# leo-stan/torch-points3d

Measured on AMD Instinct MI355X. Metric: point-clouds/sec fwd+bwd PointNet++SSG B=32 N=16384, higher is better.
Workload: dtype f32; 1 GPU; PointNet++ SSG (unet_3_ss) train step fwd+bwd+Adam, B=32 per GPU, N=16384, FEAT=3, 10 classes, pos~U[-1,1]^3 (BASELINE configs[1]); launch=hip-graph replay; geometry of step i+1 on a 2nd stream during step i, global_batch=32, points=16384, parallelism=dp1, whole clouds per rank, one flat gradient all-reduce (RCCL) per step

## Files before the change

### include/tp3d_hip.h

```cpp
#ifndef TP3D_HIP_H
#define TP3D_HIP_H

#include <stddef.h>
#include <stdint.h>

#ifdef __cplusplus
extern "C" {
#endif

#define TP3D_OK 0
#define TP3D_E_BADARG (-1)
#define TP3D_E_LAUNCH (-2)
#define TP3D_E_UNSORTED (-3)
#define TP3D_E_TOOBIG (-4)

#define TP3D_ABI_VERSION 39

int tp3d_abi_version(void);
const char *tp3d_strerror(int code);
int tp3d_last_hip_error(void);

#define TP3D_FPS_MAX_REG_POINTS 32768
int tp3d_fps_f32(const float *xyz, int B, int N, int npoint, float *scratch, int64_t *out_idx, void *stream);

// ... 272 lines not shown
                        float min_dist, float *dist2, int64_t *idx, void *workspace, size_t workspace_bytes, void *stream);
size_t tp3d_fgr_workspace_bytes(int64_t N);
int tp3d_fgr_accumulate_f32(const float *xyz, const float *xyz_target, int64_t N, int iter, void *workspace,
                            size_t workspace_bytes, void *stream);
int tp3d_fgr_solve(int64_t N, int iter, double mu_init, float *T, void *workspace, size_t workspace_bytes, void *stream);

int tp3d_segment_tile_rows(void);
int tp3d_segment_sum_chunk(void);
int tp3d_segment_transform_f32(const float *x, const float *T, const int64_t *seg, int64_t N, int64_t B, int k, int C, int ldx,
                               int ldo, int transpose, float *out, void *stream);
size_t tp3d_segment_transform_wgrad_workspace_bytes(int64_t N, int64_t B, int k);
int tp3d_segment_transform_wgrad_f32(const float *x, const float *dy, const int64_t *seg, int64_t N, int64_t B, int k, int ldx,
                                     int lddy, float *dT, void *workspace, size_t workspace_bytes, void *stream);
int tp3d_segment_bcast_cat_f32(const float *x, const float *g, const int64_t *seg, int64_t N, int64_t B, int C1, int C2, int ldx,
                               int ldg, int ldo, float *out, void *stream);
size_t tp3d_segment_sum_workspace_bytes(int64_t N, int64_t B, int C);
int tp3d_segment_sum_f32(const float *rows, const int64_t *seg, const float *scale, int64_t N, int64_t B, int col0, int C, int ld,
                         float *out, void *workspace, size_t workspace_bytes, void *stream);

#define TP3D_BOX_NMS_MAX_BOXES 4096
int tp3d_box_nms_max_boxes(void);
int tp3d_box_nms_f32(const float *boxes, const int64_t *classes, const int64_t *order, int B, int P, float overlap_threshold,
                     uint8_t *keep, void *stream);
int tp3d_box3d_iou_f64(const float *corners1, const float *corners2, int64_t n, int64_t m, double *iou, void *stream);
int tp3d_box_best_gt_f64(const float *det_corners, const int64_t *det_class, const int64_t *det_scene, int64_t D,
                         const float *gt_corners, const int64_t *gt_class, const int64_t *gt_scene_start, int64_t G, int64_t S,
                         double *ovmax, int64_t *jmax, void *stream);
int tp3d_ap_match(const int64_t *order, const int64_t *det_class, const int64_t *det_scene, int64_t D, const double *ovmax,
                  const int64_t *jmax, int64_t G, const double *thresholds, int T, uint8_t *taken, uint8_t *tp, void *stream);

int tp3d_gemm_tn_plan(int64_t M, int N, int K, int64_t *plan);
int tp3d_gemm_tn_x3_plan(int64_t M, int N, int K, int64_t *plan);
int tp3d_gemm_rows_plan(int64_t M, int N, int K, int64_t *plan);
int tp3d_bn_plan(int64_t M, int C, int pooled_ns, int64_t *plan);
int tp3d_scatter_plan(int B, int L, int nbins, int with_weights, int64_t *plan);

#ifdef __cplusplus
}
#endif
#endif
```

### torch_points3d_amd/_lib.py

```python
import collections
import ctypes
import os

import torch

from . import build as _build

_p = ctypes.c_void_p
_i = ctypes.c_int
_l = ctypes.c_int64
_f = ctypes.c_float

SIGNATURES = {
    "tp3d_fps_f32": [_p, _i, _i, _i, _p, _p, _p],
    "tp3d_ball_query_dense_f32": [_p, _p, _i, _i, _i, _f, _i, _i, _p, _p, _p, ctypes.c_size_t, _p],
    "tp3d_ball_query_partial_dense_f32": [_p, _p, _p, _p, _l, _l, _f, _i, _i, _p, _p, _p, _i, _i, _p, ctypes.c_size_t,
                                          _i, _p],
    "tp3d_three_nn_f32": [_p, _p, _i, _i, _i, _p, _p, _p],
    "tp3d_three_interpolate_fwd_f32": [_p, _p, _p, _i, _i, _i, _i, _p, _p],
    "tp3d_three_interpolate_bwd_f32": [_p, _p, _p, _i, _i, _i, _i, _p, _p, ctypes.c_size_t, _p],
    "tp3d_group_fwd_f32": [_p, _p, _i, _i, _i, _i, _i, _p, _p],
    "tp3d_group_bwd_f32": [_p, _p, _i, _i, _i, _i, _i, _p, _p, ctypes.c_size_t, _p],
    "tp3d_group_concat_fwd_f32": [_p, _p, _p, _p, _i, _i, _i, _i, _i, _i, _f, _i, _p, _p],
    "tp3d_rows_scatter_bwd_f32": [_p, _p, _p, _i, _i, _i, _i, _i, _i, _i, _p, _p, ctypes.c_size_t, _p],
# ... 54 lines not shown
    "tp3d_rsconv_msgmax_bwd_f32": [_p, _p, _p, _i, _p, _i, _p, _p, _l, _l, _l, _i, _p, _p, _p],
    "tp3d_sparse_set_build_i32": [_p, _l, _i, _i, _p, _p, _p, _p, _p, ctypes.c_size_t, _p],
    "tp3d_sparse_set_build_clouds_i32": [_p, _l, _i, _i, _i, _p, _p, _p, _p, _p, ctypes.c_size_t, _p],
    "tp3d_sparse_kmap_i32": [_p, _l, _i, _i, _i, _p, _p, _p, _l, _p, _p],
    "tp3d_sparse_kmap_mirror_i32": [_p, _l, _i, _p, _p],
    "tp3d_sparse_conv_f32": [_p, _p, _p, _l, _l, _i, _i, _i, _i, _p, _p],
    "tp3d_sparse_wgrad_f32": [_p, _p, _p, _l, _l, _i, _i, _i, _p, _p, ctypes.c_size_t, _p],
    "tp3d_sparse_conv_wide_f32": [_p, _p, _p, _l, _l, _i, _i, _i, _p, _p],
    "tp3d_sparse_wgrad_wide_f32": [_p, _p, _p, _l, _l, _i, _i, _i, _p, _p, ctypes.c_size_t, _p],
    "tp3d_scale_fuse_fwd_f32": [_p, _i, _l, _i, _i, _f, _p, _p, _p, _p, _p],
    "tp3d_scale_fuse_bwd_f32": [_p, _i, _l, _i, _i, _f, _p, _p, _p, _p, _p, _p],
    "tp3d_pv_quantize_f32": [_p, _l, _i, _p, _p],
    "tp3d_pv_trilinear_f32": [_p, _p, _l, _l, _i, _i, _p, _p],
    "tp3d_pv_invert_i32": [_p, _l, _i, _l, _p, _p, _p, ctypes.c_size_t, _p],
    "tp3d_pv_gather_f32": [_p, _p, _p, _p, _l, _i, _l, _i, _p, _p],
    "tp3d_pv_runsum_f32": [_p, _p, _p, _p, _p, _l, _i, _l, _i, _p, _p],
    "tp3d_cluster_voxel_mean_fwd_f32": [_p, _i, _p, _p, _p, _l, _l, _l, _i, _p, _p],
    "tp3d_cluster_voxel_mean_bwd_f32": [_p, _p, _p, _p, _p, _l, _l, _l, _i, _p, _p],
    "tp3d_region_grow_f32": [_p, _p, _p, _l, _p, _i, _f, _l, _p, _p, _p, _p, _p, _p, _p, ctypes.c_size_t, _p],
    "tp3d_feature_nn_f32": [_p, _p, _p, _p, _l, _l, _i, _f, _p, _p, _p, ctypes.c_size_t, _p],
    "tp3d_fgr_accumulate_f32": [_p, _p, _l, _i, _p, ctypes.c_size_t, _p],
    "tp3d_fgr_solve": [_l, _i, ctypes.c_double, _p, _p, ctypes.c_size_t, _p],
    "tp3d_segment_transform_f32": [_p, _p, _p, _l, _l, _i, _i, _i, _i, _i, _p, _p],
    "tp3d_segment_transform_wgrad_f32": [_p, _p, _p, _l, _l, _i, _i, _i, _p, _p, ctypes.c_size_t, _p],
    "tp3d_segment_bcast_cat_f32": [_p, _p, _p, _l, _l, _i, _i, _i, _i, _i, _p, _p],
    "tp3d_segment_sum_f32": [_p, _p, _p, _l, _l, _i, _i, _i, _p, _p, ctypes.c_size_t, _p],
    "tp3d_box_nms_f32": [_p, _p, _p, _i, _i, _f, _p, _p],
    "tp3d_box3d_iou_f64": [_p, _p, _l, _l, _p, _p],
    "tp3d_box_best_gt_f64": [_p, _p, _p, _l, _p, _p, _p, _l, _l, _p, _p, _p],
    "tp3d_ap_match": [_p, _p, _p, _l, _p, _p, _l, _p, _i, _p, _p, _p],
    "tp3d_gemm_tn_plan": [_l, _i, _i, _p],
    "tp3d_gemm_tn_x3_plan": [_l, _i, _i, _p],
    "tp3d_gemm_rows_plan": [_l, _i, _i, _p],
    "tp3d_bn_plan": [_l, _i, _i, _p],
    "tp3d_scatter_plan": [_i, _i, _i, _i, _p],
}
_z = ctypes.c_size_t
MISC = {
    "tp3d_abi_version": (_i, []),
    "tp3d_strerror": (ctypes.c_char_p, [_i]),
    "tp3d_last_hip_error": (_i, []),
    "tp3d_scatter_workspace_bytes": (_z, [_i, _i, _i, _i]),
    "tp3d_bn_workspace_floats": (_z, [_l, _i]),
    "tp3d_gemm_tn_workspace_floats": (_z, [_l, _i, _i]),
    "tp3d_gemm_tn_x3_workspace_floats": (_z, [_l, _i, _i]),
    "tp3d_gemm_tn_x3_serves": (_i, [_l, _i, _i]),
    "tp3d_gemm_tn_x3_red_chunks": (_i, [_l, _i, _i]),
    "tp3d_kpconv_bwd_workspace_bytes": (_z, [_l, _l]),
    "tp3d_gemm_rows_stat_floats": (_z, [_l, _i]),
    "tp3d_gemm_rows_stat_chunks": (_i, [_l, _i]),
    "tp3d_gemm_rows_narrow_chunks": (_i, [_l]),
    "tp3d_gemm_tn_bn_narrow_serves": (_i, [_l, _i, _i]),
    "tp3d_gemm_tn_bn_narrow_workspace_floats": (_z, [_l, _i, _i]),
    "tp3d_gemm_rows_bnbwd_sp_serves": (_i, [_l, _i, _i]),
    "tp3d_gemm_rows_x3_chunks": (_i, [_l, _i, _i, _i]),
    "tp3d_gemm_rows_sp_chunks": (_i, [_l, _i, _i, _i]),
    "tp3d_gemm_rows_workspace_floats": (_z, [_l, _i, _i]),
    "tp3d_kpconv_grad_workspace_bytes": (_z, [_l, _l, _i]),
    "tp3d_knn_workspace_bytes": (_z, [_i, _l, _i]),
    "tp3d_voxel_workspace_bytes": (_z, [_l]),
    "tp3d_ball_query_workspace_bytes": (_z, [_i, _l, _i]),
    "tp3d_sparse_workspace_bytes": (_z, [_l]),
    "tp3d_sparse_cloud_limit_max": (_i, []),
    "tp3d_sparse_wgrad_chunks": (_i, [_l, _i, _i, _i]),
    "tp3d_sparse_wgrad_workspace_floats": (_z, [_l, _i, _i, _i]),
    "tp3d_sparse_conv_wide_serves": (_i, [_i, _i, _i]),
# ... 225 lines not shown
```

### torch_points3d_amd/csrc/gemm_rows.hip

```cpp
#include <algorithm>

#include "tp3d_common.h"

namespace tp3d {

typedef float f32x16 __attribute__((ext_vector_type(16)));

constexpr int GR_BLOCK_T = 256;
constexpr int GR_BM = 128, GR_BK = 32;
constexpr int GR_LD = GR_BK + 4;

struct RowsEpilogue {
    const float *mean, *scale, *beta;
    float slope;
};

template <bool WIDE, int STATS>
__global__ __launch_bounds__(GR_BLOCK_T, 1) void gemm_rows_kernel(const float *__restrict__ A, const float *__restrict__ Bt,
                                                                int64_t M, int N, int K, int kchunk, int tiles_n,
                                                                int64_t items, float *__restrict__ C,
                                                                float *__restrict__ partial, RowsEpilogue epi)
{
    constexpr int BN = WIDE ? 128 : 64;
    constexpr int WR = WIDE ? 2 : 4;
    constexpr int WM = WIDE ? 2 : 1;
    constexpr int WN = 2;
    constexpr int PB = BN * (GR_BK / 4) / GR_BLOCK_T;
    __shared__ __attribute__((aligned(16))) float sA[GR_BM * GR_LD];
    __shared__ __attribute__((aligned(16))) float sB[BN * GR_LD];

    const int tid = threadIdx.x, lane = tid & 63, wave = tid >> 6;
    const int wr = WIDE ? wave >> 1 : wave, wc = WIDE ? wave & 1 : 0;
    const int l31 = lane & 31, lh = lane >> 5;
    const int kbeg = blockIdx.y * kchunk, kend = min(K, kbeg + kchunk);
    const int ksteps = (kend - kbeg + GR_BK - 1) / GR_BK;
    if (blockIdx.y > 0) C += (size_t)blockIdx.y * (size_t)M * N;

    auto decode = [&](int64_t item, int64_t &m0, int &n0, int64_t &rb) __attribute__((always_inline)) {
        const int64_t grp = item / (8 * tiles_n);
        const int rem = (int)(item % (8 * tiles_n));
        rb = grp * 8 + (rem & 7);
        m0 = rb * GR_BM;
// ... 314 lines not shown
                        pr[(size_t)N] = s2;
                        pr[(size_t)2 * N] = k;
                        pr[(size_t)3 * N] = (float)valid;
                    }
                }
            }
            if (STATS == 2) {
                if (valid > 0) have_shift = true;
                run_rows += valid;
            }
        }
        item = next_item;
        m0 = nm0;
        n0 = nn0;
        rb = nrb;
    }
    if (STATS == 2) {
        const int per = 8 * tiles_n;
        const int64_t slot = (int64_t)(blockIdx.x / per) * 8 + (blockIdx.x & 7);
#pragma unroll
        for (int j = 0; j < 2; ++j) {
            const int n = n0_first + (wc * 2 + j) * 32 + l31;
            if (lh == 0 && n < N) {
                float *pr = partial + ((size_t)(slot * 2 + wr) * 4) * N + n;
                pr[0] = run1[j];
                pr[(size_t)N] = run2[j];
                pr[(size_t)2 * N] = kshift[j];
                pr[(size_t)3 * N] = (float)run_rows;
            }
        }
    }
}


__global__ __launch_bounds__(256) void gemm_rows_sum_slabs_kernel(const float *__restrict__ slabs, int S, int64_t MN4,
                                                                   float *__restrict__ out, int N, RowsEpilogue epi)
{
    for (int64_t e = (int64_t)blockIdx.x * 256 + threadIdx.x; e < MN4; e += (int64_t)gridDim.x * 256) {
        float4 t = reinterpret_cast<const float4 *>(slabs)[e];
        for (int s = 1; s < S; ++s) {
            const float4 v = reinterpret_cast<const float4 *>(slabs + (size_t)s * MN4 * 4)[e];
            t.x += v.x;
            t.y += v.y;
            t.z += v.z;
            t.w += v.w;
        }
        if (epi.mean) {
            const int n = (int)((e * 4) % N);
            const float4 mu = *reinterpret_cast<const float4 *>(epi.mean + n), sc = *reinterpret_cast<const float4 *>(epi.scale + n);
            const float4 be = *reinterpret_cast<const float4 *>(epi.beta + n);
            t.x = (t.x - mu.x) * sc.x + be.x, t.y = (t.y - mu.y) * sc.y + be.y;
            t.z = (t.z - mu.z) * sc.z + be.z, t.w = (t.w - mu.w) * sc.w + be.w;
            t.x = t.x > 0.0f ? t.x : t.x * epi.slope, t.y = t.y > 0.0f ? t.y : t.y * epi.slope;
            t.z = t.z > 0.0f ? t.z : t.z * epi.slope, t.w = t.w > 0.0f ? t.w : t.w * epi.slope;
        }
        reinterpret_cast<float4 *>(out)[e] = t;
    }
}

}

using namespace tp3d;

namespace {
constexpr int GR_GRID = 1024;
struct RowsPlan {
    bool wide;
    int tiles_n, wave_rows;
    int64_t row_blocks, items, blocks;
    bool per_workgroup;
    int64_t chunks;
    int ksplit, kchunk;
};
RowsPlan rows_plan(int64_t M, int N, int K = 0, bool allow_split = false)
{
    RowsPlan p;
    const int rem = N % 128;
    p.wide = !(rem > 0 && rem <= 64);
    const int bn = p.wide ? 128 : 64;
    p.wave_rows = p.wide ? 2 : 4;
    p.tiles_n = (N + bn - 1) / bn;
    p.row_blocks = (M + GR_BM - 1) / GR_BM;
    const int64_t groups = (p.row_blocks + 7) / 8;
    p.items = groups * 8 * p.tiles_n;
    p.blocks = p.items < GR_GRID ? p.items : GR_GRID;
    p.per_workgroup = p.blocks == GR_GRID && GR_GRID % (8 * p.tiles_n) == 0;
    p.chunks = p.wave_rows * (p.per_workgroup ? GR_GRID / p.tiles_n : p.row_blocks);
    p.ksplit = 1;
    p.kchunk = K > 0 ? (K + GR_BK - 1) / GR_BK * GR_BK : 0;
    if (allow_split && K >= 1024 && p.items <= 128) {
        const int want = (int)((512 + p.items - 1) / p.items);
        const int by_k = K / 128;
        int s = want < by_k ? want : by_k;
        if (s > 16) s = 16;
        if (s > 1) {
            p.kchunk = ((K + s - 1) / s + GR_BK - 1) / GR_BK * GR_BK;
            p.ksplit = (K + p.kchunk - 1) / p.kchunk;
        }
    }
    return p;
}

template <bool WIDE>
int launch_rows(const RowsPlan &p, const float *A, const float *Bt, int64_t M, int N, int K, float *C, float *stat_partial,
                const RowsEpilogue &epi, hipStream_t s)
{
    const dim3 grid((unsigned)p.blocks, (unsigned)p.ksplit), block(GR_BLOCK_T);
    if (WIDE && p.ksplit == 1) {
        if (stat_partial && p.per_workgroup)
            hipLaunchKernelGGL(gemm_rows_wide_kernel<2>, grid, block, 0, s, A, Bt, M, N, K, p.tiles_n, p.items, C, stat_partial, epi);
        else if (stat_partial)
            hipLaunchKernelGGL(gemm_rows_wide_kernel<1>, grid, block, 0, s, A, Bt, M, N, K, p.tiles_n, p.items, C, stat_partial, epi);
        else
            hipLaunchKernelGGL(gemm_rows_wide_kernel<0>, grid, block, 0, s, A, Bt, M, N, K, p.tiles_n, p.items, C, stat_partial, epi);
        return check_launch();
    }
    if (stat_partial && p.per_workgroup)
        hipLaunchKernelGGL((gemm_rows_kernel<WIDE, 2>), grid, block, 0, s, A, Bt, M, N, K, p.kchunk, p.tiles_n, p.items,
                           C, stat_partial, epi);
    else if (stat_partial)
        hipLaunchKernelGGL((gemm_rows_kernel<WIDE, 1>), grid, block, 0, s, A, Bt, M, N, K, p.kchunk, p.tiles_n, p.items,
                           C, stat_partial, epi);
    else
        hipLaunchKernelGGL((gemm_rows_kernel<WIDE, 0>), grid, block, 0, s, A, Bt, M, N, K, p.kchunk, p.tiles_n, p.items,
                           C, stat_partial, epi);
    return check_launch();
}

int launch_rows_any(const RowsPlan &p, const float *A, const float *Bt, int64_t M, int N, int K, float *C,
                    float *stat_partial, const RowsEpilogue &epi, hipStream_t s)
{
    return p.wide ? launch_rows<true>(p, A, Bt, M, N, K, C, stat_partial, epi, s)
                  : launch_rows<false>(p, A, Bt, M, N, K, C, stat_partial, epi, s);
}

int rows_gemm(const float *A, const float *Bt, int64_t M, int N, int K, float *C, float *stat_partial, float *workspace,
              const RowsEpilogue &epi, hipStream_t s)
{
    const RowsEpilogue none = {nullptr, nullptr, nullptr, 1.0f};
    const RowsPlan p = rows_plan(M, N, K, !stat_partial && workspace && ((M * (int64_t)N) & 3) == 0 && (!epi.mean || (N & 3) == 0));
// ... 14 lines not shown
    const int64_t rows = p.chunks > by_block ? p.chunks : by_block;
    return (size_t)rows * 4 * (size_t)N;
}

TP3D_EXPORT int tp3d_gemm_rows_stat_chunks(int64_t M, int N)
{
    if (M <= 0 || N <= 0) return 0;
    return (int)rows_plan(M, N).chunks;
}

TP3D_EXPORT size_t tp3d_gemm_rows_workspace_floats(int64_t M, int N, int K)
{
    if (M <= 0 || N <= 0 || K <= 0) return 0;
    const RowsPlan p = rows_plan(M, N, K, true);
    return p.ksplit > 1 ? (size_t)p.ksplit * (size_t)M * (size_t)N : 0;
}

TP3D_EXPORT int tp3d_gemm_rows_plan(int64_t M, int N, int K, int64_t *plan)
{
    if (M <= 0 || N <= 0 || K < 0 || !plan) return TP3D_E_BADARG;
    const RowsPlan p = rows_plan(M, N, K, K > 0);
    plan[0] = p.tiles_n;
    plan[1] = p.row_blocks;
    plan[2] = p.items;
    plan[3] = p.blocks;
    plan[4] = p.chunks;
    plan[5] = p.per_workgroup ? 1 : 0;
    plan[6] = p.wave_rows;
    plan[7] = p.ksplit;
    plan[8] = p.wide ? 128 : 64;
    return TP3D_OK;
}

TP3D_EXPORT int tp3d_gemm_rows_f32(const float *A, const float *Bt, int64_t M, int N, int K, float *C, float *stat_partial,
                                   float *workspace, void *stream)
{
    if (M < 0 || N <= 0 || K <= 0 || (K & 3)) return TP3D_E_BADARG;
    if (M == 0) return TP3D_OK;
    if (!A || !Bt || !C) return TP3D_E_BADARG;
    const RowsEpilogue none = {nullptr, nullptr, nullptr, 1.0f};
    return rows_gemm(A, Bt, M, N, K, C, stat_partial, workspace, none, (hipStream_t)stream);
}

TP3D_EXPORT int tp3d_gemm_rows_epi_f32(const float *A, const float *Bt, int64_t M, int N, int K, const float *mean,
                                       const float *scale, const float *beta, float slope, float *C, float *workspace,
                                       void *stream)
{
    if (M < 0 || N <= 0 || K <= 0 || (K & 3)) return TP3D_E_BADARG;
    if (M == 0) return TP3D_OK;
    if (!A || !Bt || !C || !mean || !scale || !beta) return TP3D_E_BADARG;
    const RowsEpilogue epi = {mean, scale, beta, slope};
    return rows_gemm(A, Bt, M, N, K, C, nullptr, workspace, epi, (hipStream_t)stream);
}
```

### torch_points3d_amd/csrc/gemm_tn.hip

```cpp
#include <type_traits>

#include "tp3d_common.h"

namespace tp3d {

typedef float f32x16 __attribute__((ext_vector_type(16)));

constexpr int TN_BLOCK = 256;
constexpr int TN_BR_MAX = 64;

template <int WM, int WN, bool VECY, bool VECA, int GN = 2>
__global__ __launch_bounds__(TN_BLOCK) void gemm_tn_partial_kernel(const float *__restrict__ dY,
                                                                    const float *__restrict__ A, int64_t M, int N,
                                                                    int K, int64_t rows_per_split, int tiles_k,
                                                                    float *__restrict__ partial )
{
    constexpr int GK = 4 / GN;
    constexpr int TN = GN * WM * 32, TK = GK * WN * 32;
    constexpr int TN_BR = (WM * WN) % 3 == 0 ? 16 : 64 / (WM * WN);
    constexpr int LDN = TN + 4, LDK = TK + 4;
    __shared__ __attribute__((aligned(16))) float sY[TN_BR * LDN];
    __shared__ __attribute__((aligned(16))) float sA[TN_BR * LDK];

    const int tile = blockIdx.x;
    const int n0 = (tile / tiles_k) * TN, k0 = (tile % tiles_k) * TK;
    const int split = blockIdx.y;
    const int64_t r_begin = (int64_t)split * rows_per_split;
    const int64_t r_end = min(r_begin + rows_per_split, M);
    const int tid = threadIdx.x, lane = tid & 63, wave = tid >> 6;
    const int wr = wave / GK, wc = wave % GK;
    const int l31 = lane & 31, lh = lane >> 5;
    f32x16 acc[WM][WN];
#pragma unroll
    for (int i = 0; i < WM; ++i)
#pragma unroll
        for (int j = 0; j < WN; ++j)
#pragma unroll
            for (int e = 0; e < 16; ++e) acc[i][j][e] = 0.0f;


    auto load4 = [&](const float *base, int64_t r, int c, int ld, auto aligned_tag) __attribute__((always_inline)) -> float4 {
        constexpr bool aligned = decltype(aligned_tag)::value;
// ... 67 lines not shown
#pragma unroll
            for (int e = 0; e < 16; ++e) {
                const int n = n0 + (wr * WM + i) * 32 + (e & 3) + 8 * (e >> 2) + 4 * lh;
                const int k = k0 + (wc * WN + j) * 32 + l31;
                if (n < N && k < K) out[(size_t)n * K + k] = acc[i][j][e];
            }
}

constexpr int RD_E = 64, RD_S = 16;
__global__ __launch_bounds__(RD_E *RD_S) void gemm_tn_reduce_kernel(const float *__restrict__ partial, int S,
                                                                     int64_t NK, float *__restrict__ out)
{
    __shared__ float sm[RD_S][RD_E];
    const int tx = threadIdx.x % RD_E, ty = threadIdx.x / RD_E;
    const int64_t e = (int64_t)blockIdx.x * RD_E + tx;
    float acc = 0.0f;
    if (e < NK)
        for (int s = ty; s < S; s += RD_S) acc += partial[(size_t)s * NK + e];
    sm[ty][tx] = acc;
    __syncthreads();
    if (ty == 0 && e < NK) {
        float t = 0.0f;
#pragma unroll
        for (int k = 0; k < RD_S; ++k) t += sm[k][tx];
        out[e] = t;
    }
}

int tn_reduce_splits(const float *partial, int splits, int64_t NK, float *out, hipStream_t s)
{
    hipLaunchKernelGGL(gemm_tn_reduce_kernel, dim3((unsigned)((NK + RD_E - 1) / RD_E)), dim3(RD_E * RD_S), 0, s, partial, splits,
                       NK, out);
    return check_launch();
}

struct TnPlan {
    int wm, wn, gn, tn, tk, tiles_n, tiles_k, splits;
    int64_t rows_per_split;
};

static TnPlan plan_tn(int64_t M, int N, int K)
{
    TnPlan p;
    p.wm = N > 64 ? 2 : 1;
    if (K <= 64) p.wn = 1;
    else if (K <= 128) p.wn = 2;
    else if (K <= 192) p.wn = 3;
    else p.wn = ((K + 191) / 192) * 192 < ((K + 127) / 128) * 128 ? 3 : 2;
    p.gn = 2;
    if (N <= 32 && K >= 128) {
        p.gn = 1;
        p.wm = 1;
        p.wn = 1;
    }
    p.tn = 32 * p.gn * p.wm;
    p.tk = 32 * (4 / p.gn) * p.wn;
    p.tiles_n = (N + p.tn - 1) / p.tn;
    p.tiles_k = (K + p.tk - 1) / p.tk;
    const int tiles = p.tiles_n * p.tiles_k;
    int64_t want = (1024 + tiles - 1) / tiles;
    const int min_rows = 256;
    int64_t max_by_rows = (M + min_rows - 1) / min_rows;
    int64_t s = want < max_by_rows ? want : max_by_rows;
    if (s < 1) s = 1;
    if (s > 512) s = 512;
    p.rows_per_split = ((M + s - 1) / s + TN_BR_MAX - 1) / TN_BR_MAX * TN_BR_MAX;
    p.splits = (int)((M + p.rows_per_split - 1) / p.rows_per_split);
    return p;
}

static int launch_tn(const float *dY, const float *A, int64_t M, int N, int K, float *out, float *workspace, hipStream_t s)
{
    const TnPlan p = plan_tn(M, N, K);
    if (p.splits > 65535) return TP3D_E_TOOBIG;
    dim3 grid(p.tiles_n * p.tiles_k, p.splits);
    const bool vy = (N & 3) == 0, va = (K & 3) == 0;
#define TP3D_TN_LAUNCH(WM_, WN_, VY_, VA_)                                                                          \
    hipLaunchKernelGGL((gemm_tn_partial_kernel<WM_, WN_, VY_, VA_>), grid, dim3(TN_BLOCK), 0, s, dY, A, M, N, K,        \
                       p.rows_per_split, p.tiles_k, workspace)
#define TP3D_TN_ALIGN(WM_, WN_)                                                                                     \
    do {                                                                                                            \
        if (vy && va) TP3D_TN_LAUNCH(WM_, WN_, true, true);                                                         \
        else if (vy) TP3D_TN_LAUNCH(WM_, WN_, true, false);                                                         \
        else if (va) TP3D_TN_LAUNCH(WM_, WN_, false, true);                                                         \
        else TP3D_TN_LAUNCH(WM_, WN_, false, false);                                                                \
    } while (0)
    if (p.gn == 1) {
        if (vy && va) hipLaunchKernelGGL((gemm_tn_partial_kernel<1, 1, true, true, 1>), grid, dim3(TN_BLOCK), 0, s, dY, A, M, N, K,
                                         p.rows_per_split, p.tiles_k, workspace);
        else if (va) hipLaunchKernelGGL((gemm_tn_partial_kernel<1, 1, false, true, 1>), grid, dim3(TN_BLOCK), 0, s, dY, A, M, N, K,
                                        p.rows_per_split, p.tiles_k, workspace);
        else if (vy) hipLaunchKernelGGL((gemm_tn_partial_kernel<1, 1, true, false, 1>), grid, dim3(TN_BLOCK), 0, s, dY, A, M, N, K,
                                        p.rows_per_split, p.tiles_k, workspace);
        else hipLaunchKernelGGL((gemm_tn_partial_kernel<1, 1, false, false, 1>), grid, dim3(TN_BLOCK), 0, s, dY, A, M, N, K,
                                p.rows_per_split, p.tiles_k, workspace);
    } else if (p.wm == 2 && p.wn == 3) TP3D_TN_ALIGN(2, 3);
    else if (p.wn == 3) TP3D_TN_ALIGN(1, 3);
    else if (p.wm == 2 && p.wn == 2) TP3D_TN_ALIGN(2, 2);
    else if (p.wm == 2) TP3D_TN_ALIGN(2, 1);
    else if (p.wn == 2) TP3D_TN_ALIGN(1, 2);
    else TP3D_TN_ALIGN(1, 1);
// ... 42 lines not shown
```

### torch_points3d_amd/fused.py

```python
import collections

import torch
import torch.nn as nn

from . import _lib


USE_ROWS_GEMM = True


def _cl(x):
    return x.transpose(1, 2).contiguous()


def _pad4(c):
    return (c + 3) & ~3


def _slope_of(act):
    if act is None:
        return 1.0
    if isinstance(act, nn.LeakyReLU):
        return float(act.negative_slope)
    if isinstance(act, nn.ReLU):
# ... 74 lines not shown
    _lib.call("tp3d_gemm_tn_bn_narrow_f32", _lib.ptr(Y), _lib.ptr(dY_src), _lib.ptr(ls[0]), _lib.ptr(ls[2]),
              _lib.ptr(ls[3]), _lib.ptr(red[2]), _lib.ptr(red[3]), slope, _lib.ptr(A0), M, C, Kp, _lib.ptr(dW),
              _lib.ptr(nws), reverse, st)
    return dW


def gemm_tn(dY, A, x3=None, act=None, reverse=0):
    dY, A = dY.contiguous(), A.contiguous()
    M, N = dY.shape
    K = A.shape[1]
    terms = WGRAD_X3 if x3 is None else x3
    kernel = "x3" if terms and M > 0 and _lib.load().tp3d_gemm_tn_x3_serves(M, N, K) else "tn"
    if act is not None:
        if kernel != "x3":
            raise ValueError("gemm_tn(act=): only the bf16-pipe contraction forms its A operand (shape %s x %s x %s)" % (M, N, K))
        kernel = "x3_act"
    return _gemm_tn_launch(kernel, dY, A, terms, act, reverse)


def _gemm_tn_launch(kernel, dY, A, terms, act, reverse):
    dev = dY.device
    M, N = dY.shape
    K = A.shape[1]
    out = torch.empty((N, K), dtype=torch.float32, device=dev)
    ws = _lib.gemm_tn_workspace(M, N, K, dev, x3=kernel != "tn")
    with _lib.on_device(dev):
        if kernel == "x3_act":
            _lib.call("tp3d_gemm_tn_x3_act_f32", _lib.ptr(dY), _lib.ptr(A), _lib.ptr(act[0]), _lib.ptr(act[1]), _lib.ptr(act[2]),
                      float(act[3]), M, N, K, int(terms), _lib.ptr(out), _lib.ptr(ws), int(reverse), _lib.stream_ptr(dev))
        elif kernel == "x3":
            _lib.call("tp3d_gemm_tn_x3_f32", _lib.ptr(dY), _lib.ptr(A), M, N, K, int(terms), _lib.ptr(out), _lib.ptr(ws), int(reverse),
                      _lib.stream_ptr(dev))
        else:
            _lib.call("tp3d_gemm_tn_f32", _lib.ptr(dY), _lib.ptr(A), M, N, K, _lib.ptr(out), _lib.ptr(ws),
                      _lib.stream_ptr(dev))
    return out


SKINNY_MAX = 32
SKINNY_MIN_ROWS = 32768


def gemm_skinny(A, W):
    dev = A.device
    A, W = A.contiguous(), W.contiguous()
    M, K = A.shape
    N = W.shape[0]
    Y = torch.empty((M, N), dtype=torch.float32, device=dev)
    with _lib.on_device(dev):
        _lib.call("tp3d_gemm_skinny_f32", _lib.ptr(A), _lib.ptr(W), M, N, K, K, _lib.ptr(Y), _lib.stream_ptr(dev))
    return Y


def _is_skinny(M, a, b):
    return M >= SKINNY_MIN_ROWS and a <= SKINNY_MAX and b <= SKINNY_MAX


def gemm_rows(A, Bt, want_stats=False):
    dev = A.device
    M, K = A.shape
    N = Bt.shape[0]
    Bm = Bt.contiguous()
    C = torch.empty((M, N), dtype=torch.float32, device=dev)
    part, slabs = None, None
    h = _lib.load()
    if want_stats:
        part = _lib.workspace("gemm_rows_stats", 4 * h.tp3d_gemm_rows_stat_floats(M, N), dev)
    else:
        n = h.tp3d_gemm_rows_workspace_floats(M, N, K)
        if n:
            slabs = _lib.workspace("gemm_rows_slabs", 4 * n, dev)
    with _lib.on_device(dev):
        _lib.call("tp3d_gemm_rows_f32", _lib.ptr(A), _lib.ptr(Bm), M, N, K, _lib.ptr(C), _lib.ptr(part), _lib.ptr(slabs),
                  _lib.stream_ptr(dev))
    return C, part


def _finalize_stats(part, M, C, gamma, beta, bn, dev, st, chunks=None):
    stats = torch.empty((4, C), dtype=torch.float32, device=dev)
    if chunks is None:
        chunks = _lib.load().tp3d_gemm_rows_stat_chunks(M, C)
    _lib.call("tp3d_bn_finalize_f32", _lib.ptr(part), chunks, M, C, float(bn.eps),
              float(bn.momentum), _lib.ptr(gamma), _lib.ptr(beta), _lib.ptr(bn.running_mean), _lib.ptr(bn.running_var),
              _lib.ptr(bn.num_batches_tracked), _lib.ptr(stats[0]), _lib.ptr(stats[1]), _lib.ptr(stats[2]), _lib.ptr(stats[3]), st)
    _note_training_pass(bn)
    return stats


def _note_training_pass(bn):
    bn._tp3d_train_passes = getattr(bn, "_tp3d_train_passes", 0) + 1


_replay_epoch = 0


def note_graph_replay():
    global _replay_epoch
    _replay_epoch += 1


def eval_state_key(tensors, bns):
    return (tuple((t.data_ptr(), t._version) for t in tensors)
            + tuple(getattr(bn, "_tp3d_train_passes", 0) for bn in bns) + (_replay_epoch,))


ROWS_GEMM_MIN_COLS = 32
ROWS_GEMM_WITHOUT_STATS = True
ROWS_GEMM_EPILOGUE = True
ROWS_GEMM_NARROW = True
CHAIN_MIN_ROWS = 32768


def _rows_gemm_serves(cout):
    if not USE_ROWS_GEMM or cout < ROWS_GEMM_MIN_COLS:
        return False
    return ROWS_GEMM_NARROW or not (0 < cout % 128 <= 64)


def _bn_stats(Y, M, C, gamma, beta, bn, training, dev, st, bias=None):
    key = None
    if not training:
        key = eval_state_key((gamma, beta, bn.running_mean, bn.running_var) + ((bias,) if bias is not None else ()), (bn,))
        hit = getattr(bn, "_tp3d_eval_stats", None)
        if hit is not None and hit[0] == key:
            return hit[1]
    stats = torch.empty((4, C), dtype=torch.float32, device=dev)
    ws = _lib.bn_workspace(M, C, dev)
    _lib.call("tp3d_bn_stats_f32", _lib.ptr(Y), M, C, float(bn.eps), float(bn.momentum), _lib.ptr(gamma), _lib.ptr(beta),
              _lib.ptr(bn.running_mean), _lib.ptr(bn.running_var), _lib.ptr(bn.num_batches_tracked) if training else None,
              int(training), _lib.ptr(stats[0]), _lib.ptr(stats[1]), _lib.ptr(stats[2]), _lib.ptr(stats[3]), _lib.ptr(ws), st)
    if training:
        _note_training_pass(bn)
    if key is not None:
        if bias is not None:
            stats[0].sub_(bias.detach())
        bn._tp3d_eval_stats = (key, stats)
# ... 37 lines not shown
    want_stats = training and _lib.load().tp3d_gemm_rows_workspace_floats(M, Cout, Kp) == 0
    if rows and ROWS_GEMM_EPILOGUE and not training and not pool_ns and ROWS_GEMM_WITHOUT_STATS and not want_grad:
        return "rows_epi", False
    if rows and (want_stats or ROWS_GEMM_WITHOUT_STATS):
        return "rows", want_stats
    if skinny:
        return "skinny", False
    return "library", False


class _LinearBNAct(torch.autograd.Function):

    @staticmethod
    def forward(ctx, A, weight, gamma, beta, bn, slope, pool_ns, grad_enabled, bias=None):
        dev = A.device
        A = A.contiguous()
        M, Kp = A.shape
        Cout = weight.shape[0]
        W2 = weight.reshape(Cout, -1)
        Cin = W2.shape[1]
        if Kp != Cin:
            W2 = torch.nn.functional.pad(W2, (0, Kp - Cin))
        training = bn.training
        st = _lib.stream_ptr(dev)
        path, want_stats = _layer_route(M, Kp, Cout, training, pool_ns, grad_enabled and any(ctx.needs_input_grad))
        if path in ("skinny_bnact", "rows_epi"):
            with _lib.on_device(dev):
                stats = _bn_stats(A, M, Cout, gamma, beta, bn, False, dev, st, bias)
                out = torch.empty((M, Cout), dtype=torch.float32, device=dev)
                if path == "skinny_bnact":
                    _lib.call("tp3d_gemm_skinny_bnact_f32", _lib.ptr(A), _lib.ptr(W2.contiguous()), M, Cout, Kp, Kp,
                              _lib.ptr(stats[0]), _lib.ptr(stats[2]), _lib.ptr(stats[3]), slope, _lib.ptr(out), st)
                else:
                    n = _lib.load().tp3d_gemm_rows_workspace_floats(M, Cout, Kp)
                    slabs = _lib.workspace("gemm_rows_slabs", 4 * n, dev) if n else None
                    _lib.call("tp3d_gemm_rows_epi_f32", _lib.ptr(A), _lib.ptr(W2.contiguous()), M, Cout, Kp, _lib.ptr(stats[0]),
                              _lib.ptr(stats[2]), _lib.ptr(stats[3]), slope, _lib.ptr(out), _lib.ptr(slabs), st)
            return out.view(M // pool_ns, pool_ns, Cout).max(1)[0] if pool_ns else out
        part = None
        if path == "rows":
            Y, part = gemm_rows(A, W2, want_stats=want_stats)
        elif path == "skinny":
            Y = gemm_skinny(A, W2)
        else:
            Y = torch.mm(A, W2.t())
        with _lib.on_device(dev):
            if part is not None:
                stats = _finalize_stats(part, M, Cout, gamma, beta, bn, dev, st)
            else:
                stats = _bn_stats(Y, M, Cout, gamma, beta, bn, training, dev, st, bias)
            out, arg = _bn_act_out(Y, stats, slope, pool_ns, st)
        if training and bias is not None:
            bn.running_mean.add_(bias.detach(), alpha=float(bn.momentum))
        ctx.save_for_backward(A, W2, Y, stats, arg)
        ctx.cfg = (slope, pool_ns, training, tuple(weight.shape), Cin, bias is not None)
        return out

    @staticmethod
    def backward(ctx, grad_out):
        A, W2, Y, stats, arg = ctx.saved_tensors
        slope, pool_ns, training, wshape, Cin, has_bias = ctx.cfg
        dev = grad_out.device
        grad_out = grad_out.contiguous()
        M, Cout = Y.shape
        need_A, need_W, need_bias = ctx.needs_input_grad[0], ctx.needs_input_grad[1], ctx.needs_input_grad[-1]
        with _lib.on_device(dev):
# ... 20 lines not shown
        dev = A0.device
        A0 = A0.contiguous()
        M, K0 = A0.shape
        st = _lib.stream_ptr(dev)
        L = len(layers)
        training = layers[0][0].training
        need = ctx.needs_input_grad
        first = len(need) - len(params)
        plan = _plan_chain(M, K0, [params[3 * l].shape[0] for l in range(L)], pool_ns, grad_enabled and any(need), need[0],
                           need[first::3], grad_cols)
        Ys, stats, W2s, cins, acts = [], [], [], [], [None] * (L - 1)
        with _lib.on_device(dev):
            for l, ((bn, slope), p) in enumerate(zip(layers, plan)):
                weight, gamma, beta = params[3 * l], params[3 * l + 1], params[3 * l + 2]
                Cout = weight.shape[0]
                W2 = weight.reshape(Cout, -1)
                Kp = K0 if l == 0 else Ys[-1].shape[1]
                cins.append(W2.shape[1])
                if W2.shape[1] != Kp:
                    W2 = torch.nn.functional.pad(W2, (0, Kp - W2.shape[1]))
                W2 = W2.contiguous()
                Y = torch.empty((M, Cout), dtype=torch.float32, device=dev)
                part = None
                if training:
                    nbytes = 16 * p.chunks * Cout if p.reverse is not None else 4 * _lib.load().tp3d_gemm_rows_stat_floats(M, Cout)
                    part = _lib.workspace("gemm_rows_stats", nbytes, dev)
                if p.kernel == "narrow":
                    _lib.call("tp3d_gemm_rows_narrow_f32", _lib.ptr(A0), _lib.ptr(W2), M, Cout, Kp, _lib.ptr(Y), _lib.ptr(part), p.reverse, st)
                elif p.kernel in ("rows", "bn_act_rows"):
                    src = A0
                    if l:
                        src = _bn_act_out(Ys[-1], stats[-1], layers[l - 1][1], 0, st)[0]
                        acts[l - 1] = src if p.keep_act else None
                    _lib.call("tp3d_gemm_rows_f32", _lib.ptr(src), _lib.ptr(W2), M, Cout, Kp, _lib.ptr(Y), _lib.ptr(part), None, st)
                else:
                    if l == 0:
                        ident = _identity_stats(Kp, dev)
                        src, mean, scale, shift, pslope = A0, ident[0], ident[1], ident[0], 1.0
                    else:
                        ps = stats[-1]
                        src, mean, scale, shift, pslope = Ys[-1], ps[0], ps[2], ps[3], layers[l - 1][1]
                        acts[l - 1] = torch.empty((M, Kp), dtype=torch.float32, device=dev) if p.keep_act else None
                    _lib.call("tp3d_gemm_rows_bnact_sp_f32" if p.kernel == "sp" else "tp3d_gemm_rows_bnact_x3_f32", _lib.ptr(src),
                              _lib.ptr(mean), _lib.ptr(scale), _lib.ptr(shift), pslope, _lib.ptr(W2), M, Cout, Kp, _lib.ptr(Y),
                              _lib.ptr(part), _lib.ptr(acts[l - 1]) if l else None, p.reverse, st)
                if training:
                    stats.append(_finalize_stats(part, M, Cout, gamma, beta, bn, dev, st, p.chunks))
                else:
                    stats.append(_bn_stats(Y, M, Cout, gamma, beta, bn, False, dev, st))
                Ys.append(Y)
                W2s.append(W2)
            out, arg = _bn_act_out(Ys[-1], stats[-1], layers[-1][1], pool_ns, st)
        ctx.save_for_backward(A0, arg, *Ys, *stats, *W2s, *(acts if plan[0].bwd else []))
        ctx.cfg = (L, pool_ns, training, [s_ for _, s_ in layers], [tuple(params[3 * l].shape) for l in range(L)], cins)
        ctx.plan = plan
        return out

    @staticmethod
    def backward(ctx, grad_out):
        L, pool_ns, training, slopes, wshapes, cins = ctx.cfg
        saved = ctx.saved_tensors
        A0, arg = saved[0], saved[1]
        Ys, stats, W2s = saved[2:2 + L], saved[2 + L:2 + 2 * L], saved[2 + 2 * L:2 + 3 * L]
        dev = grad_out.device
        st = _lib.stream_ptr(dev)
        M = A0.shape[0]
# ... 398 lines not shown
```

Before: 4568 point-clouds/s.

## Add small-tile rows GEMM and narrower TN tiles for low-occupancy shapes

```diff
diff --git a/include/tp3d_hip.h b/include/tp3d_hip.h
--- a/include/tp3d_hip.h
+++ b/include/tp3d_hip.h
@@ -328,6 +328,8 @@
 int tp3d_gemm_tn_plan(int64_t M, int N, int K, int64_t *plan);
 int tp3d_gemm_tn_x3_plan(int64_t M, int N, int K, int64_t *plan);
 int tp3d_gemm_rows_plan(int64_t M, int N, int K, int64_t *plan);
+int tp3d_gemm_rows_small_plan(int64_t M, int N, int K, int64_t *plan);
+int tp3d_set_few_row_tiles(int on);
 int tp3d_bn_plan(int64_t M, int C, int pooled_ns, int64_t *plan);
 int tp3d_scatter_plan(int B, int L, int nbins, int with_weights, int64_t *plan);
 
diff --git a/torch_points3d_amd/_lib.py b/torch_points3d_amd/_lib.py
--- a/torch_points3d_amd/_lib.py
+++ b/torch_points3d_amd/_lib.py
@@ -110,6 +110,8 @@
     "tp3d_gemm_tn_plan": [_l, _i, _i, _p],
     "tp3d_gemm_tn_x3_plan": [_l, _i, _i, _p],
     "tp3d_gemm_rows_plan": [_l, _i, _i, _p],
+    "tp3d_gemm_rows_small_plan": [_l, _i, _i, _p],
+    "tp3d_set_few_row_tiles": [_i],
     "tp3d_bn_plan": [_l, _i, _i, _p],
     "tp3d_scatter_plan": [_i, _i, _i, _i, _p],
 }
diff --git a/torch_points3d_amd/csrc/gemm_plans.h b/torch_points3d_amd/csrc/gemm_plans.h
--- /dev/null
+++ b/torch_points3d_amd/csrc/gemm_plans.h
@@ -0,0 +1,115 @@
+#pragma once
+#include <stdint.h>
+
+namespace tp3d {
+
+inline int g_few_row_tiles = 1;
+
+constexpr int GR_BM = 128, GR_BK = 32;
+constexpr int GR_GRID = 1024;
+constexpr int GR_SMALL_ITEMS = 256;
+
+struct RowsPlan {
+    bool wide;
+    int tiles_n, wave_rows;
+    int64_t row_blocks, items, blocks;
+    bool per_workgroup;
+    int64_t chunks;
+    int ksplit, kchunk;
+};
+inline RowsPlan rows_plan(int64_t M, int N, int K = 0, bool allow_split = false)
+{
+    RowsPlan p;
+    const int rem = N % 128;
+    p.wide = !(rem > 0 && rem <= 64);
+    const int bn = p.wide ? 128 : 64;
+    p.wave_rows = p.wide ? 2 : 4;
+    p.tiles_n = (N + bn - 1) / bn;
+    p.row_blocks = (M + GR_BM - 1) / GR_BM;
+    const int64_t groups = (p.row_blocks + 7) / 8;
+    p.items = groups * 8 * p.tiles_n;
+    p.blocks = p.items < GR_GRID ? p.items : GR_GRID;
+    p.per_workgroup = p.blocks == GR_GRID && GR_GRID % (8 * p.tiles_n) == 0;
+    p.chunks = p.wave_rows * (p.per_workgroup ? GR_GRID / p.tiles_n : p.row_blocks);
+    p.ksplit = 1;
+    p.kchunk = K > 0 ? (K + GR_BK - 1) / GR_BK * GR_BK : 0;
+    if (allow_split && K >= 1024 && p.items <= 128) {
+        const int want = (int)((512 + p.items - 1) / p.items);
+        const int by_k = K / 128;
+        int s = want < by_k ? want : by_k;
+        if (s > 16) s = 16;
+        if (s > 1) {
+            p.kchunk = ((K + s - 1) / s + GR_BK - 1) / GR_BK * GR_BK;
+            p.ksplit = (K + p.kchunk - 1) / p.kchunk;
+        }
+    }
+    return p;
+}
+
+struct RowsSmallPlan {
+    bool routed;
+    int64_t items, blocks;
+};
+inline RowsSmallPlan rows_small_plan(const RowsPlan &p)
+{
+    RowsSmallPlan s;
+    s.routed = g_few_row_tiles != 0 && p.wide && p.ksplit == 1 && p.items <= GR_SMALL_ITEMS;
+    s.items = s.blocks = s.routed ? 4 * p.items : 0;
+    return s;
+}
+
+constexpr int TN_BR_MAX = 64;
+constexpr int TN_FILL = 256;
+
+struct TnPlan {
+    int wm, wn, gn, tn, tk, tiles_n, tiles_k, splits;
+    int64_t rows_per_split;
+};
+
+inline void tn_set_tile(TnPlan &p, int N, int K)
+{
+    p.tn = 32 * p.gn * p.wm;
+    p.tk = 32 * (4 / p.gn) * p.wn;
+    p.tiles_n = (N + p.tn - 1) / p.tn;
+    p.tiles_k = (K + p.tk - 1) / p.tk;
+}
+
+inline TnPlan plan_tn(int64_t M, int N, int K)
+{
+    TnPlan p;
+    p.wm = N > 64 ? 2 : 1;
+    if (K <= 64) p.wn = 1;
+    else if (K <= 128) p.wn = 2;
+    else if (K <= 192) p.wn = 3;
+    else p.wn = ((K + 191) / 192) * 192 < ((K + 127) / 128) * 128 ? 3 : 2;
+    p.gn = 2;
+    if (N <= 32 && K >= 128) {
+        p.gn = 1;
+        p.wm = 1;
+        p.wn = 1;
+    }
+    tn_set_tile(p, N, K);
+    const int tiles = p.tiles_n * p.tiles_k;
+    int64_t want = (1024 + tiles - 1) / tiles;
+    const int min_rows = 256;
+    int64_t max_by_rows = (M + min_rows - 1) / min_rows;
+    int64_t s = want < max_by_rows ? want : max_by_rows;
+    if (s < 1) s = 1;
+    if (s > 512) s = 512;
+    p.rows_per_split = ((M + s - 1) / s + TN_BR_MAX - 1) / TN_BR_MAX * TN_BR_MAX;
+    p.splits = (int)((M + p.rows_per_split - 1) / p.rows_per_split);
+    if (g_few_row_tiles != 0 && p.gn == 2 && p.wn != 3 && (int64_t)tiles * p.splits < TN_FILL) {
+        const int cand[3][2] = {{2, 1}, {1, 2}, {1, 1}};
+        const int wm0 = p.wm, wn0 = p.wn;
+        for (int c = 0; c < 3; ++c) {
+            if (cand[c][0] > wm0 || cand[c][1] > wn0 || (cand[c][0] == wm0 && cand[c][1] == wn0)) continue;
+            p.wm = cand[c][0];
+            p.wn = cand[c][1];
+            tn_set_tile(p, N, K);
+            if ((int64_t)p.tiles_n * p.tiles_k * p.splits >= TN_FILL) break;
+        }
+    }
+    return p;
+}
+
+}
diff --git a/torch_points3d_amd/csrc/gemm_rows.hip b/torch_points3d_amd/csrc/gemm_rows.hip
--- a/torch_points3d_amd/csrc/gemm_rows.hip
+++ b/torch_points3d_amd/csrc/gemm_rows.hip
@@ -1,5 +1,6 @@
 #include <algorithm>
 
+#include "gemm_plans.h"
 #include "tp3d_common.h"
 
 namespace tp3d {
@@ -7,7 +8,6 @@
 typedef float f32x16 __attribute__((ext_vector_type(16)));
 
 constexpr int GR_BLOCK_T = 256;
-constexpr int GR_BM = 128, GR_BK = 32;
 constexpr int GR_LD = GR_BK + 4;
 
 struct RowsEpilogue {
@@ -388,6 +388,149 @@
     }
 }
 
+template <int STATS>
+__global__ __launch_bounds__(GR_BLOCK_T, 4) void gemm_rows_small_kernel(const float *__restrict__ A, const float *__restrict__ Bt,
+                                                                 int64_t M, int N, int K, int tiles_n, float *__restrict__ C,
+                                                                 float *__restrict__ partial, RowsEpilogue epi)
+{
+    constexpr int BT = 64;
+    __shared__ __attribute__((aligned(16))) float sA[2][BT * GR_LD];
+    __shared__ __attribute__((aligned(16))) float sB[2][BT * GR_LD];
+    __shared__ float sStat[STATS ? 2 : 1][3][64];
+
+    const int tid = threadIdx.x, lane = tid & 63, wave = __builtin_amdgcn_readfirstlane(tid >> 6);
+    const int wr = wave >> 1, wc = wave & 1;
+    const int l31 = lane & 31, lh = lane >> 5;
+    const int ksteps = (K + GR_BK - 1) / GR_BK;
+    const int tail_groups = (K - (ksteps - 1) * GR_BK + 7) / 8;
+
+    const int per = 32 * tiles_n;
+    const int rem = (int)(blockIdx.x % per);
+    const int64_t rb = (int64_t)(blockIdx.x / per) * 8 + (rem & 7);
+    if (rb * GR_BM >= M) return;
+    const int half = (rem >> 3) & 1;
+    const int n0 = (rem >> 4) * BT;
+    const int64_t m0 = rb * GR_BM + half * BT;
+
+    const int frow = tid >> 3, fk4 = (tid & 7) * 4;
+    const bool oka0 = m0 + frow < M, oka1 = m0 + frow + 32 < M, okb0 = n0 + frow < N, okb1 = n0 + frow + 32 < N;
+    const float *pa0 = A + min(m0 + frow, M - 1) * K, *pa1 = A + min(m0 + frow + 32, M - 1) * K;
+    const float *pb0 = Bt + (size_t)min(n0 + frow, N - 1) * K, *pb1 = Bt + (size_t)min(n0 + frow + 32, N - 1) * K;
+    struct Stage {
+        float4 a0, a1, b0, b1;
+    };
+    auto fetch = [&](Stage &s, int k0) __attribute__((always_inline)) {
+        const int kk = min(k0 + fk4, K - 4);
+        s.a0 = *reinterpret_cast<const float4 *>(pa0 + kk);
+        s.a1 = *reinterpret_cast<const float4 *>(pa1 + kk);
+        s.b0 = *reinterpret_cast<const float4 *>(pb0 + kk);
+        s.b1 = *reinterpret_cast<const float4 *>(pb1 + kk);
+    };
+    auto keep = [](bool ok, const float4 &v) __attribute__((always_inline)) {
+        return make_float4(ok ? v.x : 0.f, ok ? v.y : 0.f, ok ? v.z : 0.f, ok ? v.w : 0.f);
+    };
+    auto stash = [&](const Stage &s, int buf, int k0) __attribute__((always_inline)) {
+        const bool kin = k0 + fk4 < K;
+        float *da = &sA[buf][frow * GR_LD + fk4], *db = &sB[buf][frow * GR_LD + fk4];
+        *reinterpret_cast<float4 *>(da) = keep(kin && oka0, s.a0);
+        *reinterpret_cast<float4 *>(da + 32 * GR_LD) = keep(kin && oka1, s.a1);
+        *reinterpret_cast<float4 *>(db) = keep(kin && okb0, s.b0);
+        *reinterpret_cast<float4 *>(db + 32 * GR_LD) = keep(kin && okb1, s.b1);
+    };
+    f32x16 acc;
+#pragma unroll
+    for (int e = 0; e < 16; ++e) acc[e] = 0.0f;
+    auto compute = [&](int buf, int ng ) __attribute__((always_inline)) {
+#pragma unroll
+        for (int g = 0; g < GR_BK / 8; ++g) {
+            if (g < ng) {
+                const float4 a = *reinterpret_cast<const float4 *>(&sA[buf][(wr * 32 + l31) * GR_LD + g * 8 + lh * 4]);
+                const float4 b = *reinterpret_cast<const float4 *>(&sB[buf][(wc * 32 + l31) * GR_LD + g * 8 + lh * 4]);
+                acc = __builtin_amdgcn_mfma_f32_32x32x2f32(a.x, b.x, acc, 0, 0, 0);
+                acc = __builtin_amdgcn_mfma_f32_32x32x2f32(a.y, b.y, acc, 0, 0, 0);
+                acc = __builtin_amdgcn_mfma_f32_32x32x2f32(a.z, b.z, acc, 0, 0, 0);
+                acc = __builtin_amdgcn_mfma_f32_32x32x2f32(a.w, b.w, acc, 0, 0, 0);
+            }
+        }
+    };
+
+    Stage s0, s1;
+    fetch(s0, 0);
+    fetch(s1, GR_BK);
+    int ks = 0;
+#pragma unroll 1
+    for (; ks + 1 < ksteps; ks += 2) {
+        stash(s0, 0, ks * GR_BK);
+        fetch(s0, (ks + 2) * GR_BK);
+        __syncthreads();
+        compute(0, GR_BK / 8);
+        stash(s1, 1, (ks + 1) * GR_BK);
+        fetch(s1, (ks + 3) * GR_BK);
+        __syncthreads();
+        compute(1, ks + 2 < ksteps ? GR_BK / 8 : tail_groups);
+    }
+    if (ksteps & 1) {
+        stash(s0, 0, ks * GR_BK);
+        __syncthreads();
+        compute(0, tail_groups);
+    }
+
+    const int n = n0 + wc * 32 + l31;
+    {
+        float emu = 0.0f, esc = 1.0f, ebe = 0.0f;
+        if (epi.mean && n < N) emu = epi.mean[n], esc = epi.scale[n], ebe = epi.beta[n];
+#pragma unroll
+        for (int e = 0; e < 16; ++e) {
+            const int64_t m = m0 + wr * 32 + (e & 3) + 8 * (e >> 2) + 4 * lh;
+            float v = acc[e];
+            if (epi.mean) {
+                v = (v - emu) * esc + ebe;
+                v = v > 0.0f ? v : v * epi.slope;
+            }
+            if (m < M && n < N) C[m * N + n] = v;
+        }
+    }
+    if (STATS != 0) {
+        const int valid = (int)min((int64_t)BT, max((int64_t)0, M - m0));
+        const float pad = (float)(BT - valid);
+        float k = 0.0f, s1 = 0.0f, s2 = 0.0f;
+        if (wr == 0) {
+            k = __shfl(acc[0], l31);
+#pragma unroll
+            for (int e = 0; e < 16; ++e) {
+                const float d = acc[e] - k;
+                s1 += d;
+                s2 += d * d;
+            }
+            sStat[wc][0][lane] = k;
+            sStat[wc][1][lane] = s1;
+            sStat[wc][2][lane] = s2;
+        }
+        __syncthreads();
+        if (wr == 1) {
+            k = sStat[wc][0][lane];
+            s1 = sStat[wc][1][lane];
+            s2 = sStat[wc][2][lane];
+#pragma unroll
+            for (int e = 0; e < 16; ++e) {
+                const float d = acc[e] - k;
+                s1 += d;
+                s2 += d * d;
+            }
+            s1 += __shfl_xor(s1, 32);
+            s2 += __shfl_xor(s2, 32);
+            s1 += pad * k;
+            s2 -= pad * (k * k);
+            if (lh == 0 && n < N) {
+                float *pr = partial + ((size_t)(rb * 2 + half) * 4) * N + n;
+                pr[0] = s1;
+                pr[(size_t)N] = s2;
+                pr[(size_t)2 * N] = k;
+                pr[(size_t)3 * N] = (float)valid;
+            }
+        }
+    }
+}
 
 __global__ __launch_bounds__(256) void gemm_rows_sum_slabs_kernel(const float *__restrict__ slabs, int S, int64_t MN4,
                                                                    float *__restrict__ out, int N, RowsEpilogue epi)
@@ -419,49 +562,19 @@
 using namespace tp3d;
 
 namespace {
-constexpr int GR_GRID = 1024;
-struct RowsPlan {
-    bool wide;
-    int tiles_n, wave_rows;
-    int64_t row_blocks, items, blocks;
-    bool per_workgroup;
-    int64_t chunks;
-    int ksplit, kchunk;
-};
-RowsPlan rows_plan(int64_t M, int N, int K = 0, bool allow_split = false)
-{
-    RowsPlan p;
-    const int rem = N % 128;
-    p.wide = !(rem > 0 && rem <= 64);
-    const int bn = p.wide ? 128 : 64;
-    p.wave_rows = p.wide ? 2 : 4;
-    p.tiles_n = (N + bn - 1) / bn;
-    p.row_blocks = (M + GR_BM - 1) / GR_BM;
-    const int64_t groups = (p.row_blocks + 7) / 8;
-    p.items = groups * 8 * p.tiles_n;
-    p.blocks = p.items < GR_GRID ? p.items : GR_GRID;
-    p.per_workgroup = p.blocks == GR_GRID && GR_GRID % (8 * p.tiles_n) == 0;
-    p.chunks = p.wave_rows * (p.per_workgroup ? GR_GRID / p.tiles_n : p.row_blocks);
-    p.ksplit = 1;
-    p.kchunk = K > 0 ? (K + GR_BK - 1) / GR_BK * GR_BK : 0;
-    if (allow_split && K >= 1024 && p.items <= 128) {
-        const int want = (int)((512 + p.items - 1) / p.items);
-        const int by_k = K / 128;
-        int s = want < by_k ? want : by_k;
-        if (s > 16) s = 16;
-        if (s > 1) {
-            p.kchunk = ((K + s - 1) / s + GR_BK - 1) / GR_BK * GR_BK;
-            p.ksplit = (K + p.kchunk - 1) / p.kchunk;
-        }
-    }
-    return p;
-}
-
 template <bool WIDE>
 int launch_rows(const RowsPlan &p, const float *A, const float *Bt, int64_t M, int N, int K, float *C, float *stat_partial,
                 const RowsEpilogue &epi, hipStream_t s)
 {
     const dim3 grid((unsigned)p.blocks, (unsigned)p.ksplit), block(GR_BLOCK_T);
+    if (const RowsSmallPlan sp = rows_small_plan(p); WIDE && sp.routed) {
+        const dim3 sgrid((unsigned)sp.blocks);
+        if (stat_partial)
+            hipLaunchKernelGGL(gemm_rows_small_kernel<1>, sgrid, block, 0, s, A, Bt, M, N, K, p.tiles_n, C, stat_partial, epi);
+        else
+            hipLaunchKernelGGL(gemm_rows_small_kernel<0>, sgrid, block, 0, s, A, Bt, M, N, K, p.tiles_n, C, stat_partial, epi);
+        return check_launch();
+    }
     if (WIDE && p.ksplit == 1) {
         if (stat_partial && p.per_workgroup)
             hipLaunchKernelGGL(gemm_rows_wide_kernel<2>, grid, block, 0, s, A, Bt, M, N, K, p.tiles_n, p.items, C, stat_partial, epi);
@@ -542,6 +655,23 @@
     return TP3D_OK;
 }
 
+TP3D_EXPORT int tp3d_set_few_row_tiles(int on)
+{
+    g_few_row_tiles = on != 0;
+    return TP3D_OK;
+}
+
+TP3D_EXPORT int tp3d_gemm_rows_small_plan(int64_t M, int N, int K, int64_t *plan)
+{
+    if (M <= 0 || N <= 0 || K < 0 || !plan) return TP3D_E_BADARG;
+    const RowsSmallPlan a = rows_small_plan(rows_plan(M, N, K, false)), b = rows_small_plan(rows_plan(M, N, K, K > 0));
+    plan[0] = a.routed ? a.items : b.items;
+    plan[1] = a.routed ? a.blocks : b.blocks;
+    plan[2] = a.routed ? 1 : 0;
+    plan[3] = b.routed ? 1 : 0;
+    return TP3D_OK;
+}
+
 TP3D_EXPORT int tp3d_gemm_rows_f32(const float *A, const float *Bt, int64_t M, int N, int K, float *C, float *stat_partial,
                                    float *workspace, void *stream)
 {
diff --git a/torch_points3d_amd/csrc/gemm_tn.hip b/torch_points3d_amd/csrc/gemm_tn.hip
--- a/torch_points3d_amd/csrc/gemm_tn.hip
+++ b/torch_points3d_amd/csrc/gemm_tn.hip
@@ -1,5 +1,6 @@
 #include <type_traits>
 
+#include "gemm_plans.h"
 #include "tp3d_common.h"
 
 namespace tp3d {
@@ -7,7 +8,6 @@
 typedef float f32x16 __attribute__((ext_vector_type(16)));
 
 constexpr int TN_BLOCK = 256;
-constexpr int TN_BR_MAX = 64;
 
 template <int WM, int WN, bool VECY, bool VECA, int GN = 2>
 __global__ __launch_bounds__(TN_BLOCK) void gemm_tn_partial_kernel(const float *__restrict__ dY,
@@ -141,41 +141,6 @@
     hipLaunchKernelGGL(gemm_tn_reduce_kernel, dim3((unsigned)((NK + RD_E - 1) / RD_E)), dim3(RD_E * RD_S), 0, s, partial, splits,
                        NK, out);
     return check_launch();
-}
-
-struct TnPlan {
-    int wm, wn, gn, tn, tk, tiles_n, tiles_k, splits;
-    int64_t rows_per_split;
-};
-
-static TnPlan plan_tn(int64_t M, int N, int K)
-{
-    TnPlan p;
-    p.wm = N > 64 ? 2 : 1;
-    if (K <= 64) p.wn = 1;
-    else if (K <= 128) p.wn = 2;
-    else if (K <= 192) p.wn = 3;
-    else p.wn = ((K + 191) / 192) * 192 < ((K + 127) / 128) * 128 ? 3 : 2;
-    p.gn = 2;
-    if (N <= 32 && K >= 128) {
-        p.gn = 1;
-        p.wm = 1;
-        p.wn = 1;
-    }
-    p.tn = 32 * p.gn * p.wm;
-    p.tk = 32 * (4 / p.gn) * p.wn;
-    p.tiles_n = (N + p.tn - 1) / p.tn;
-    p.tiles_k = (K + p.tk - 1) / p.tk;
-    const int tiles = p.tiles_n * p.tiles_k;
-    int64_t want = (1024 + tiles - 1) / tiles;
-    const int min_rows = 256;
-    int64_t max_by_rows = (M + min_rows - 1) / min_rows;
-    int64_t s = want < max_by_rows ? want : max_by_rows;
-    if (s < 1) s = 1;
-    if (s > 512) s = 512;
-    p.rows_per_split = ((M + s - 1) / s + TN_BR_MAX - 1) / TN_BR_MAX * TN_BR_MAX;
-    p.splits = (int)((M + p.rows_per_split - 1) / p.rows_per_split);
-    return p;
 }
 
 static int launch_tn(const float *dY, const float *A, int64_t M, int N, int K, float *out, float *workspace, hipStream_t s)
diff --git a/torch_points3d_amd/fused.py b/torch_points3d_amd/fused.py
--- a/torch_points3d_amd/fused.py
+++ b/torch_points3d_amd/fused.py
@@ -130,6 +130,7 @@
             _lib.call("tp3d_gemm_tn_x3_f32", _lib.ptr(dY), _lib.ptr(A), M, N, K, int(terms), _lib.ptr(out), _lib.ptr(ws), int(reverse),
                       _lib.stream_ptr(dev))
         else:
+            sync_few_row_tiles()
             _lib.call("tp3d_gemm_tn_f32", _lib.ptr(dY), _lib.ptr(A), M, N, K, _lib.ptr(out), _lib.ptr(ws),
                       _lib.stream_ptr(dev))
     return out
@@ -162,6 +163,7 @@
     C = torch.empty((M, N), dtype=torch.float32, device=dev)
     part, slabs = None, None
     h = _lib.load()
+    sync_few_row_tiles()
     if want_stats:
         part = _lib.workspace("gemm_rows_stats", 4 * h.tp3d_gemm_rows_stat_floats(M, N), dev)
     else:
@@ -200,6 +202,18 @@
 def eval_state_key(tensors, bns):
     return (tuple((t.data_ptr(), t._version) for t in tensors)
             + tuple(getattr(bn, "_tp3d_train_passes", 0) for bn in bns) + (_replay_epoch,))
+
+
+FEW_ROW_TILES = 1
+_few_row_pushed = None
+
+
+def sync_few_row_tiles():
+    global _few_row_pushed
+    v = int(FEW_ROW_TILES)
+    if v != _few_row_pushed:
+        _lib.load().tp3d_set_few_row_tiles(v)
+        _few_row_pushed = v
 
 
 ROWS_GEMM_MIN_COLS = 32
@@ -303,6 +317,7 @@
                     _lib.call("tp3d_gemm_skinny_bnact_f32", _lib.ptr(A), _lib.ptr(W2.contiguous()), M, Cout, Kp, Kp,
                               _lib.ptr(stats[0]), _lib.ptr(stats[2]), _lib.ptr(stats[3]), slope, _lib.ptr(out), st)
                 else:
+                    sync_few_row_tiles()
                     n = _lib.load().tp3d_gemm_rows_workspace_floats(M, Cout, Kp)
                     slabs = _lib.workspace("gemm_rows_slabs", 4 * n, dev) if n else None
                     _lib.call("tp3d_gemm_rows_epi_f32", _lib.ptr(A), _lib.ptr(W2.contiguous()), M, Cout, Kp, _lib.ptr(stats[0]),
@@ -389,6 +404,7 @@
                     if l:
                         src = _bn_act_out(Ys[-1], stats[-1], layers[l - 1][1], 0, st)[0]
                         acts[l - 1] = src if p.keep_act else None
+                    sync_few_row_tiles()
                     _lib.call("tp3d_gemm_rows_f32", _lib.ptr(src), _lib.ptr(W2), M, Cout, Kp, _lib.ptr(Y), _lib.ptr(part), None, st)
                 else:
                     if l == 0:
```

Result: faster. 4688 point-clouds/s, median of 6 (+2.6%).
